# MrTornado24/FENeRF

Hardware: AMD Instinct MI355X
Metric: rays/s/GPU forward render (128x128, 24+24 samples, H=256 FiLM-SIREN + 32x96^3 grid) (higher is better)
Workload: dtype f16x3 (error-compensated fp16 MFMA, fp32 accumulate; fp32-class accuracy); 1 GPU; configs[1]: CelebA_double_semantic_texture_embedding_256_dim_96 generator, 128x128, 24+24 hierarchical samples, batch 1/GPU, forward-only render, procedural weights; img_size=128, num_steps=24, batch_per_gpu=1

## Files before the change

### fenerf_amd/csrc/fenerf_siren_f16w.hip

```cpp
#include <hip/hip_runtime.h>

#include <type_traits>

#include "fenerf_composite_ray.h"
#include "fenerf_film.h"
#include "fenerf_internal.h"
#include "fenerf_layout.h"
#include "fenerf_trig.h"


namespace fenerf {
namespace w16 {

typedef float f32x4 __attribute__((ext_vector_type(4)));
typedef _Float16 half8 __attribute__((ext_vector_type(8)));
typedef _Float16 half4 __attribute__((ext_vector_type(4)));
typedef _Float16 half2 __attribute__((ext_vector_type(2)));

#define MFMA16W(a, b, c) __builtin_amdgcn_mfma_f32_16x16x32_f16((a), (b), (c), 0, 0, 0)
#define MFMA32W(a, b, c) __builtin_amdgcn_mfma_f32_16x16x4f32((a), (b), (c), 0, 0, 0)

constexpr int CH = FENERF_CH;
constexpr int DPF = FENERF_DPF;
constexpr int NSLOT = FENERF_NSLOT;
constexpr int NWAVE = 8;
static_assert(CH == NWAVE, "one 1-KiB A operand per wave and chunk");
static_assert(NSLOT >= DPF + 2, "a slot is refilled two barriers after its last reader issued its reads");

__device__ __forceinline__ half8 as_half8(const float4& v) { return __builtin_bit_cast(half8, v); }
__device__ __forceinline__ unsigned lds_addr(const void* p) {
  return (unsigned)(size_t)(const __attribute__((address_space(3))) char*)p;
}
__device__ __forceinline__ void glds_1k(const char* g_lane, unsigned lds_uniform) {
  asm volatile(
      "s_mov_b32 m0, %1\n\t"
      "s_nop 0\n\t"
      "global_load_lds_dwordx4 %0, off"
      :
      : "v"(g_lane), "s"(lds_uniform)
      : "memory");
}
__device__ __forceinline__ void glds_1k_s(const void* g_uniform, unsigned voff, unsigned lds_uniform) {
  asm volatile(
      "s_mov_b32 m0, %2\n\t"
      "s_nop 0\n\t"
      "global_load_lds_dwordx4 %0, %1"
      :
      : "v"(voff), "s"(g_uniform), "s"(lds_uniform)
      : "memory");
}
__device__ __forceinline__ int opaque(int v) {
  asm volatile("" : "+v"(v));
  return v;
}
#define WAIT_VMCNT(n) asm volatile("s_waitcnt vmcnt(%0)" ::"n"(n) : "memory")
template <class T>
__device__ __forceinline__ T* uniform_ptr(T* p) {
  const unsigned long long v = reinterpret_cast<unsigned long long>(p);
  const unsigned lo = __builtin_amdgcn_readfirstlane((unsigned)v), hi = __builtin_amdgcn_readfirstlane((unsigned)(v >> 32));
  return reinterpret_cast<T*>(((unsigned long long)hi << 32) | lo);
}
template <int MODE> struct TapeW { const char* base; };
typedef unsigned u32x4 __attribute__((ext_vector_type(4)));
#ifndef FENERF_ST_POLICY
#define FENERF_ST_POLICY "nt"
#endif
__device__ __forceinline__ void st_f4_nt(const void* g_uniform, unsigned voff, const f32x4& v) {
  asm volatile("global_store_dwordx4 %0, %1, %2 " FENERF_ST_POLICY "\n\ts_nop 1" : : "v"(voff), "v"(v), "s"(g_uniform) : "memory");
}
__device__ __forceinline__ void st_u4_nt(const void* g_uniform, unsigned voff, const u32x4& v) {
  asm volatile("global_store_dwordx4 %0, %1, %2 " FENERF_ST_POLICY "\n\ts_nop 1" : : "v"(voff), "v"(v), "s"(g_uniform) : "memory");
}
struct TapeQ { unsigned q[4]; };
__device__ __forceinline__ unsigned phase_u16(float theta) {
  const float v = __builtin_amdgcn_fractf(theta) * 65536.f;
  const unsigned c = __builtin_bit_cast(unsigned, v + 8388608.f) & 0xffffu;
  return !(__builtin_fabsf(theta) < __builtin_inff()) ? TAPE16_NONFINITE : (c == TAPE16_NONFINITE ? (v < 65535.f ? 0xfffeu : 0u) : c);
}
#define LDS_FENCE() asm volatile("" ::: "memory")
#ifndef FENERF_WAVE_HALF_COPIES
#define FENERF_WAVE_HALF_COPIES 1
#endif
#ifndef FENERF_EXP_DEPHASE
#define FENERF_EXP_DEPHASE 0
#endif

struct WStream {
  bool skip;
  unsigned long long g_next;
  unsigned voff;
  unsigned ring_lds;
  const char* ring_lane;
  bool early;
};

__device__ __forceinline__ void ws_issue(WStream& w, int slot) {
  const unsigned m0 = w.ring_lds + (unsigned)slot * (CH * 1024);
  if (!w.skip)
    asm volatile(
        "s_mov_b32 m0, %2\n\t"
        "s_nop 0\n\t"
        "global_load_lds_dwordx4 %0, %1"
        :
        : "v"(w.voff), "s"(w.g_next), "s"(m0)
        : "memory");
  w.g_next += CH * 1024;
}

struct AK { float4 hi[2], lo[2]; };
__device__ __forceinline__ void ws_read_lo(AK& a, const WStream& w, int slot, int spl) {
  const float4* p = reinterpret_cast<const float4*>(w.ring_lane + slot * (CH * 1024) + spl * 4096);
  a.lo[0] = p[1 * 64]; a.lo[1] = p[3 * 64];
}
__device__ __forceinline__ void ws_read_hi(AK& a, const WStream& w, int slot, int spl) {
  const float4* p = reinterpret_cast<const float4*>(w.ring_lane + slot * (CH * 1024) + spl * 4096);
  a.hi[0] = p[0 * 64]; a.hi[1] = p[2 * 64];
}
template <bool LO = true>
__device__ __forceinline__ AK ws_read(const WStream& w, int slot, int spl) {
  AK a;
  if (LO) ws_read_lo(a, w, slot, spl);
  else { a.lo[0] = make_float4(0.f, 0.f, 0.f, 0.f); a.lo[1] = a.lo[0]; }
  ws_read_hi(a, w, slot, spl);
  return a;
}

__device__ __forceinline__ void ws_step(WStream& w, int i, bool early) {
  const bool sync = (i & 1) == 0;
  if (sync) {
    WAIT_VMCNT(DPF - 3);
    __builtin_amdgcn_s_barrier();
  }
  LDS_FENCE();
  if (early)
    ws_issue(w, (i + DPF) % NSLOT);
}
__device__ __forceinline__ void ws_issue_late(WStream& w, int i, bool early) {
  if (!early) ws_issue(w, (i + DPF) % NSLOT);
}

template <bool LO = true>
__device__ __forceinline__ void kstep_mfma(f32x4 (&acc)[2], const AK& a, const half8& bh, const half8& bl) {
  if (LO) {
    acc[0] = MFMA16W(as_half8(a.lo[0]), bh, acc[0]);
    acc[1] = MFMA16W(as_half8(a.lo[1]), bh, acc[1]);
  }
  acc[0] = MFMA16W(as_half8(a.hi[0]), bl, acc[0]);
  acc[1] = MFMA16W(as_half8(a.hi[1]), bl, acc[1]);
  acc[0] = MFMA16W(as_half8(a.hi[0]), bh, acc[0]);
  acc[1] = MFMA16W(as_half8(a.hi[1]), bh, acc[1]);
}

struct FilmQ { float2 f, p; };
template <int PF4>
__device__ __forceinline__ FilmQ epi_load(int nbp, int piece, const float* film) {
  const int rt = piece >> 1, pc = piece & 1;
  FilmQ q;
  q.f = *reinterpret_cast<const float2*>(film + 32 * nbp + 8 * rt + 2 * pc);
  q.p = *reinterpret_cast<const float2*>(film + PF4 + 32 * nbp + 8 * rt + 2 * pc);
  return q;
}
template <int KS, int SAVE>
__device__ __forceinline__ void epi_compute(const f32x4 (&acc)[2], int nbp, int piece, const FilmQ& q, half8 (&yh)[KS],
                                            half8 (&yl)[KS], TapeW<SAVE> tw, int tile_odd, TapeQ& tq) {
  const int rt = piece >> 1, pc = piece & 1;
  const float2 f = q.f, p = q.p;
  if (SAVE == 1 && pc == 0) {
    const int lo = opaque((int)(threadIdx.x & 63));
    const unsigned toff = (unsigned)(((2 * (lo >> 5)) * 64 + ((lo >> 4) & 1) * 32 + 16 * tile_odd + (lo & 15)) * 16);
    st_f4_nt(tw.base + (nbp * 4 + rt) * 1024, toff, acc[rt]);
  }
  const float th0 = __builtin_fmaf(f.x, acc[rt][2 * pc + 0], p.x), th1 = __builtin_fmaf(f.y, acc[rt][2 * pc + 1], p.y);
  if (SAVE == 2) {
    tq.q[piece] = __builtin_amdgcn_perm(phase_u16(th1), phase_u16(th0), 0x05040100u);
    if (piece == 3) {
      const int lo = opaque((int)(threadIdx.x & 63));
      const u32x4 v = {tq.q[0], tq.q[1], tq.q[2], tq.q[3]};
      st_u4_nt(tw.base + nbp * 2048, (unsigned)(1024 * tile_odd + 16 * lo), v);
    }
  }
  const float s0 = sin2pi(th0);
  const float s1 = sin2pi(th1);
  const _Float16 h0 = (_Float16)__builtin_fmaf(s0, F16_ACT_SCALE, 0.f), h1 = (_Float16)__builtin_fmaf(s1, F16_ACT_SCALE, 0.f);
  half2 hp = {h0, h1}, lp = {(_Float16)__builtin_fmaf(s0, F16_ACT_SCALE, -(float)h0), (_Float16)__builtin_fmaf(s1, F16_ACT_SCALE, -(float)h1)};
  asm volatile("" : "+v"(hp), "+v"(lp));
  const int s = 4 * rt + 2 * pc;
  yh[nbp][s] = hp[0]; yh[nbp][s + 1] = hp[1];
  yl[nbp][s] = lp[0]; yl[nbp][s + 1] = lp[1];
}
template <int KS, int PF4, int SAVE>
__device__ __forceinline__ void epi_piece(const f32x4 (&acc)[2], int nbp, int piece, const float* film, half8 (&yh)[KS],
                                          half8 (&yl)[KS], TapeW<SAVE> tw, int tile_odd, TapeQ& tq) {
  epi_compute<KS, SAVE>(acc, nbp, piece, epi_load<PF4>(nbp, piece, film), yh, yl, tw, tile_odd, tq);
}
template <int KS, int PF4, int SAVE>
__device__ __forceinline__ void epi_all(const f32x4 (&acc)[2], int nbp, const float* film, half8 (&yh)[KS], half8 (&yl)[KS],
                                        TapeW<SAVE> tw, int tile_odd) {
  TapeQ tq;
#pragma unroll
  for (int pc = 0; pc < 4; ++pc) epi_piece<KS, PF4, SAVE>(acc, nbp, pc, film, yh, yl, tw, tile_odd, tq);
}

struct APipe { AK c, n; };
struct FilmQ2 { FilmQ q[4]; };
template <bool LOR = true, bool LOM = true, int PH = -1, class BOP, class LOADQ, class PIECE>
__device__ __forceinline__ void chunk_step(f32x4 (&acc)[2], APipe& a, WStream& ws, int i, int sp0, BOP bop, LOADQ loadq, PIECE piece) {
  const bool early = PH < 0 ? ws.early : PH == 0;
  constexpr int PSPL = (PH == 1 && FENERF_EXP_DEPHASE == 1) ? 0 : 1;
  ws_step(ws, i, early);
  FilmQ2 fq;
#pragma unroll
  for (int spl = 0; spl < 2; ++spl) {
    if (spl == 1) ws_issue_late(ws, i, early);
    if (spl == 0) loadq(fq);
    const AK nn = ws_read<LOR>(ws, (i + 1) % NSLOT, spl);
    __builtin_amdgcn_sched_barrier(0);
    half8 bh, bl;
    if (bop(sp0 + spl, bh, bl)) kstep_mfma<LOR && LOM>(acc, a.c, bh, bl);
    if (spl == PSPL) piece(fq);
    a.c = a.n;
    a.n = nn;
    __builtin_amdgcn_sched_barrier(0);
  }
}
template <bool LO = true, int PH = -1>
__device__ __forceinline__ void chunk_skip(APipe& a, WStream& ws, int i) {
  const bool early = PH < 0 ? ws.early : PH == 0;
  ws_step(ws, i, early);
  ws_issue_late(ws, i, early);
  a.c = ws_read<LO>(ws, (i + 1) % NSLOT, 0);
  a.n = ws_read<LO>(ws, (i + 1) % NSLOT, 1);
  __builtin_amdgcn_sched_barrier(0);
}

template <int QB>
__device__ __forceinline__ void piece_range(int qc, int& p0, int& p1) {
  constexpr int QBE = QB < 4 ? QB : 4;
  if (qc >= QBE) { p0 = p1 = 0; return; }
  p0 = 4 * qc / QBE;
  p1 = 4 * (qc + 1) / QBE;
}

template <bool FUSED> struct FuseArgs {};
template <> struct FuseArgs<true> {
  int rays_per_group, octs_per_group;
  long long groups, total_rays;
  float* z_fine;
  float* out_fine;
  CompositeParams coarse;
  CompositeParams final_;
};
#ifndef FENERF_EXP_RAY_PHASE
#define FENERF_EXP_RAY_PHASE 2
#endif
#ifndef FENERF_EXP_FUSED_MAXM
#define FENERF_EXP_FUSED_MAXM 128
#endif
constexpr int FUSED_MAXM = FENERF_EXP_FUSED_MAXM;

template <int H, bool GRID, int SAVE, bool FUSED = false, int TERMS2 = 0>
__global__ __launch_bounds__(512, 2) void siren16w_kernel(SirenParams P, int n_geo, int n_color, int n_lab, int C, FuseArgs<FUSED> F) {
  static_assert(!(FUSED && SAVE != 0), "the fused render is the no-grad path");
  static_assert(TERMS2 == 0 || (SAVE == 0 && !FUSED), "the reduced-precision forwards are plain no-grad evaluations");
  constexpr bool LOR = TERMS2 != 1;
  constexpr bool LOC = TERMS2 == 0;
  constexpr int NB = H / 32, KS = H / 32;
  constexpr int QB = (KS + 1) / 2;
  constexpr int C0_KS = KS + (GRID ? 1 : 0) + 1;
  constexpr int C0_QB = (2 * (2 * KS + (GRID ? 2 : 0) + 1) + CH - 1) / CH;
  constexpr int SQ_CHUNKS = pad_stage(NB * QB * CH) / CH;
  constexpr int C0_CHUNKS = pad_stage(NB * C0_QB * CH) / CH;
  constexpr int HEAD_CHUNKS = pad_stage(QB * CH) / CH;
  extern __shared__ __attribute__((aligned(16))) float4 smem[];

  if (P.clk && threadIdx.x == 0) {
    P.clk[(size_t)blockIdx.x * 4 + 0] = __builtin_amdgcn_s_memtime();
    P.clk[(size_t)blockIdx.x * 4 + 1] = __builtin_amdgcn_s_memrealtime();
  }
  const int lane = threadIdx.x & 63;
  const int wave = __builtin_amdgcn_readfirstlane(threadIdx.x >> 6);
  const int n = lane & 15, g = lane >> 4;
  const int L = n_geo + n_color;
  const int stage_f4 = (16 * C + 3) / 4;
  char* lds = reinterpret_cast<char*>(smem);
  char* ring = lds;
  constexpr int FILM_F = H * 4 < 1024 ? 1024 : H * 4;
  constexpr int FILM_BYTES = 2 * FILM_F;
  char* film_base = lds + NSLOT * CH * 1024 + wave * (2 * FILM_BYTES);
  float* l0_lds = reinterpret_cast<float*>(lds + NSLOT * CH * 1024 + NWAVE * 2 * FILM_BYTES);
  float* cst = l0_lds + NB * 256;
  float* stage = cst + 80 + wave * stage_f4 * 4;
  float4* ext_wave = reinterpret_cast<float4*>(cst + 80 + NWAVE * stage_f4 * 4) + wave * 256;

  for (int i = threadIdx.x; i < NB * 256; i += 512) l0_lds[i] = P.stream[i];
  if (threadIdx.x < 32) {
    cst[threadIdx.x] = P.consts[CONST_FILM_BIAS + (size_t)2 * L * H + threadIdx.x];
    cst[32 + threadIdx.x] = P.consts[CONST_HEAD_BIAS + threadIdx.x];
  } else if (threadIdx.x < 36) {
    cst[64 + threadIdx.x - 32] = P.consts[CONST_FILM_BIAS + (size_t)2 * L * H + threadIdx.x];
    cst[68 + threadIdx.x - 32] = P.consts[CONST_RGB_BIAS + threadIdx.x - 32];
  }
  CompositeParams* ray_par = reinterpret_cast<CompositeParams*>(reinterpret_cast<float4*>(cst + 80 + NWAVE * stage_f4 * 4) + NWAVE * 256);
  if constexpr (FUSED) {
    constexpr int NW = (int)(sizeof(CompositeParams) / 4);
    static_assert(sizeof(CompositeParams) % 4 == 0 && NW <= 256, "copied one dword per thread");
    const int t = threadIdx.x & 255;
    const unsigned* src = reinterpret_cast<const unsigned*>(threadIdx.x < 256 ? &F.coarse : &F.final_);
    if (t < NW) reinterpret_cast<unsigned*>(ray_par + (threadIdx.x >> 8))[t] = src[t];
  }
  WAIT_VMCNT(0);
  __syncthreads();

  WStream ws;
  {
    const int spl = wave >> 2, rt = (wave >> 1) & 1, hl = wave & 1;
    const int gi = n >> 2, r = n & 3;
    const int row = 16 * (gi >> 1) + 4 * (gi & 1) + 8 * rt + r;
    const int e_old = 2 * (2 * spl + (g >> 1)) + hl;
    ws.voff = e_old * 1024 + ((g & 1) * 32 + row) * 16;
  }
  const unsigned long long g_stream = reinterpret_cast<unsigned long long>(P.stream + P.ring_offset_floats);
  ws.g_next = g_stream;
  ws.ring_lds = __builtin_amdgcn_readfirstlane(lds_addr(ring) + wave * 1024);
  ws.ring_lane = ring + lane * 16;
  ws.early = wave < NWAVE / 2;
  ws.skip = TERMS2 == 1 && (wave & 1);

  const long long ntiles = (P.P + 15) / 16;
  const long long nocts = (ntiles + NWAVE - 1) / NWAVE;
  int opg = 1;
  long long nunits = nocts;
  if constexpr (FUSED) { opg = F.octs_per_group; nunits = F.groups; }
  const int nblk = gridDim.x;
  const int nx = nblk < 8 ? nblk : 8;
  const int xcd = blockIdx.x % nx, bi = blockIdx.x / nx;
  const int blocks_in_x = nblk / nx + (xcd < nblk % nx ? 1 : 0);
  const long long o_begin = nunits * xcd / nx, o_end = nunits * (xcd + 1) / nx;

  if (P.raw_fg && o_begin + bi < o_end) {
    const long long p_first = (o_begin + bi) * opg * (NWAVE * 16);
    long long p_last = o_end * opg * (NWAVE * 16) - 1;
    if (p_last >= P.P) p_last = P.P - 1;
    film_prep_prologue(P, p_first / P.pts_per_image, p_last / P.pts_per_image, H, n_geo, n_color);
  }

#pragma unroll
  for (int i = 0; i < DPF; ++i) ws_issue(ws, i);
  WAIT_VMCNT(DPF - 1);
  __builtin_amdgcn_s_barrier();
  LDS_FENCE();
  if (wave >= NWAVE / 2) __builtin_amdgcn_s_setprio(1);
  APipe a_cur;
  a_cur.c = ws_read<LOR>(ws, 0, 0);
  a_cur.n = ws_read<LOR>(ws, 0, 1);


  for (long long unit = o_begin + bi; unit < o_end; unit += blocks_in_x) {
  const int nsub = FUSED ? 2 * opg : 1;
#pragma unroll 1
  for (int sub = 0; sub < nsub; ++sub) {
    const bool fine_pass = FUSED && sub >= opg;
    const long long oct = FUSED ? unit * opg + (fine_pass ? sub - opg : sub) : unit;
    const float* z_src = P.z;
    float* out_dst = P.out;
    if constexpr (FUSED) {
      if (fine_pass) { z_src = F.z_fine; out_dst = F.out_fine; }
    }
    ws.g_next = g_stream + (unsigned long long)DPF * (CH * 1024);
    const long long tile = oct * NWAVE + wave;
    long long pt = tile * 16 + n;
    if (pt >= P.P) pt = P.P - 1;
    const long long img = __builtin_amdgcn_readfirstlane((int)(pt / P.pts_per_image));
    float px, py, pz, dx, dy, dz;
    if (P.points) {
      px = P.points[pt * 3 + 0]; py = P.points[pt * 3 + 1]; pz = P.points[pt * 3 + 2];
      if (P.pdirs) { dx = P.pdirs[pt * 3 + 0]; dy = P.pdirs[pt * 3 + 1]; dz = P.pdirs[pt * 3 + 2]; }
      else { dx = 0.f; dy = 0.f; dz = -1.f; }
    } else {
      const long long ray = pt / P.n_per_ray;
      const float zz = z_src[pt];
      const float ox = P.origins[ray * 3 + 0], oy = P.origins[ray * 3 + 1], oz = P.origins[ray * 3 + 2];
      dx = P.dirs[ray * 3 + 0]; dy = P.dirs[ray * 3 + 1]; dz = P.dirs[ray * 3 + 2];
      px = __fadd_rn(ox, __fmul_rn(dx, zz)); py = __fadd_rn(oy, __fmul_rn(dy, zz)); pz = __fadd_rn(oz, __fmul_rn(dz, zz));
      if (P.lock_view) { dx = 0.f; dy = 0.f; dz = -1.f; }
    }
    const float qx = px * P.box_scale, qy = py * P.box_scale, qz = pz * P.box_scale;
    constexpr int TL = SAVE == 2 ? H * 64 : H * 128;
    const int tile_odd = (int)(tile & 1);
    const char* tape_tile = SAVE ? uniform_ptr(reinterpret_cast<const char*>(P.tape) + (size_t)(tile >> 1) * L * TL) : nullptr;
    auto tape_of = [&](int layer) {
      TapeW<SAVE> t{SAVE ? uniform_ptr(tape_tile + (size_t)layer * TL) : nullptr};
      if (SAVE) asm volatile("s_nop 4" ::: "memory");
      return t;
    };

    const float* fp_img = P.fp + (size_t)img * L * H;
    const float* pp_img = P.pp + (size_t)img * L * H;
    auto film_issue = [&](int layer) {
      const unsigned dst = __builtin_amdgcn_readfirstlane(lds_addr(film_base) + (layer & 1) * FILM_BYTES);
      const float* gf = fp_img + (size_t)layer * H;
      const float* gp = pp_img + (size_t)layer * H;
      const unsigned vo = (unsigned)opaque(lane) * 16;
      for (int off = 0; off < H * 4; off += 1024) {
        glds_1k_s(reinterpret_cast<const char*>(gf) + off, vo, dst + off);
        glds_1k_s(reinterpret_cast<const char*>(gp) + off, vo, dst + FILM_F + off);
      }
    };
    film_issue(0);
    if (L > 1) film_issue(1);

    float e[8];
#pragma unroll
    for (int i = 0; i < 8; ++i) e[i] = 0.f;
    if (GRID) {
      const int ch0 = 16 * (g & 1) + 8 * (g >> 1);
      const float ix = ((qx + 1.f) / 2.f) * (float)(P.gw - 1);
      const float iy = ((qy + 1.f) / 2.f) * (float)(P.gh - 1);
      const float iz = ((qz + 1.f) / 2.f) * (float)(P.gd - 1);
      const float x0 = floorf(ix), y0 = floorf(iy), z0 = floorf(iz);
#pragma unroll
      for (int c = 0; c < 8; ++c) {
        const int cz = c >> 2, cy = (c >> 1) & 1, cx = c & 1;
        const float xi = x0 + cx, yi = y0 + cy, zi = z0 + cz;
        const float wx = cx ? (ix - x0) : (x0 + 1.f - ix);
        const float wy = cy ? (iy - y0) : (y0 + 1.f - iy);
        const float wz = cz ? (iz - z0) : (z0 + 1.f - iz);
        const float wgt = wx * wy * wz;
        const bool ok = xi >= 0.f && xi <= (float)(P.gw - 1) && yi >= 0.f && yi <= (float)(P.gh - 1) && zi >= 0.f &&
                        zi <= (float)(P.gd - 1);
        if (ok) {
          const long long vox = ((long long)(int)zi * P.gh + (int)yi) * P.gw + (int)xi;
          const float4* gp = reinterpret_cast<const float4*>(P.grid + vox * 32 + ch0);
#pragma unroll
          for (int q = 0; q < 2; ++q) {
            const float4 v = gp[q];
            e[4 * q + 0] += v.x * wgt; e[4 * q + 1] += v.y * wgt; e[4 * q + 2] += v.z * wgt; e[4 * q + 3] += v.w * wgt;
          }
        }
      }
    }
    if (SAVE && GRID) {
      float4* ep = reinterpret_cast<float4*>(P.tape_e + pt * 32 + 16 * (g & 1) + 8 * (g >> 1));
      ep[0] = make_float4(e[0], e[1], e[2], e[3]);
      ep[1] = make_float4(e[4], e[5], e[6], e[7]);
    }
    {
      half8 eh, el, dh, dl;
#pragma unroll
      for (int t = 0; t < 8; ++t) {
        const float v = e[t] * F16_ACT_SCALE;
        const _Float16 hh = (_Float16)v;
        eh[t] = hh; el[t] = (_Float16)(v - (float)hh);
      }
      const float d3[3] = {dx * F16_ACT_SCALE, dy * F16_ACT_SCALE, dz * F16_ACT_SCALE};
#pragma unroll
      for (int t = 0; t < 8; ++t) { dh[t] = (_Float16)0.f; dl[t] = (_Float16)0.f; }
#pragma unroll
      for (int t = 0; t < 3; ++t) {
        const float v = g == 0 ? d3[t] : 0.f;
        const _Float16 hh = (_Float16)v;
        dh[t] = hh; dl[t] = (_Float16)(v - (float)hh);
      }
      float4* ext = ext_wave + lane;
      ext[0] = __builtin_bit_cast(float4, eh); ext[64] = __builtin_bit_cast(float4, el);
      ext[128] = __builtin_bit_cast(float4, dh); ext[192] = __builtin_bit_cast(float4, dl);
    }
    WAIT_VMCNT(0);
    LDS_FENCE();

    auto film_lane = [&](int layer) -> const float* {
      const int gq = opaque(lane) >> 4;
      return reinterpret_cast<const float*>(film_base + (layer & 1) * FILM_BYTES) + 16 * (gq >> 1) + 4 * (gq & 1);
    };

    half8 xh[KS], xl[KS];
    {
      const float b = g == 0 ? qx : (g == 1 ? qy : (g == 2 ? qz : 0.f));
      const int gi = n >> 2, r = n & 3;
      const float* wl = l0_lds + ((g & 1) * 32 + 16 * (gi >> 1) + 4 * (gi & 1) + r) * 4 + (g >> 1);
      const TapeW<SAVE> tw0 = tape_of(0);
#pragma unroll
      for (int nb = 0; nb < NB; ++nb) {
        f32x4 acc[2];
#pragma unroll
        for (int rt = 0; rt < 2; ++rt) {
          const f32x4 z4 = {0.f, 0.f, 0.f, 0.f};
          acc[rt] = MFMA32W(wl[nb * 256 + 8 * rt * 4], b, z4);
        }
        epi_all<KS, FILM_F / 4, SAVE>(acc, nb, film_lane(0), xh, xl, tw0, tile_odd);
      }
    }
    auto film_layer = [&](auto ph_c, int l) {
      constexpr int PH = decltype(ph_c)::value;
      const float* ff = film_lane(l);
      const TapeW<SAVE> tw = tape_of(l);
      half8 yh[KS], yl[KS];
      if (l + 1 < L) film_issue(l + 1);
      if (SQ_CHUNKS < DPF + 2) WAIT_VMCNT(0);
      if (l == n_geo) {
        const float4* ext = ext_wave + opaque(lane);
        auto bop0 = [&](int sp, half8& bh, half8& bl) -> bool {
          if (sp < KS) { bh = xh[sp]; bl = xl[sp]; return true; }
          if (GRID && sp == KS) { bh = as_half8(ext[0]); bl = as_half8(ext[64]); return true; }
          if (sp == C0_KS - 1) { bh = as_half8(ext[128]); bl = as_half8(ext[192]); return true; }
          return false;
        };
        f32x4 acc_prev[2] = {{0.f, 0.f, 0.f, 0.f}, {0.f, 0.f, 0.f, 0.f}};
        TapeQ tq;
#pragma unroll
        for (int nb = 0; nb < NB; ++nb) {
          f32x4 acc[2] = {{0.f, 0.f, 0.f, 0.f}, {0.f, 0.f, 0.f, 0.f}};
#pragma unroll
          for (int qc = 0; qc < C0_QB; ++qc) {
            chunk_step<LOR, LOC, PH>(acc, a_cur, ws, nb * C0_QB + qc, 2 * qc, bop0, [&](FilmQ2& fq) {
              if (nb > 0) {
                int p0, p1;
                piece_range<C0_QB>(qc, p0, p1);
#pragma unroll
                for (int pc = 0; pc < 4; ++pc)
                  if (pc >= p0 && pc < p1) fq.q[pc] = epi_load<FILM_F / 4>(nb - 1, pc, ff);
              }
            }, [&](const FilmQ2& fq) {
              if (nb > 0) {
                int p0, p1;
                piece_range<C0_QB>(qc, p0, p1);
#pragma unroll
                for (int pc = 0; pc < 4; ++pc)
                  if (pc >= p0 && pc < p1) epi_compute<KS, SAVE>(acc_prev, nb - 1, pc, fq.q[pc], yh, yl, tw, tile_odd, tq);
              }
            });
          }
          acc_prev[0] = acc[0]; acc_prev[1] = acc[1];
        }
#pragma unroll
        for (int i = NB * C0_QB; i < C0_CHUNKS; ++i) chunk_skip<LOR, PH>(a_cur, ws, i);
        epi_all<KS, FILM_F / 4, SAVE>(acc_prev, NB - 1, ff, yh, yl, tw, tile_odd);
        {
          f32x4 acc[2] = {{0.f, 0.f, 0.f, 0.f}, {0.f, 0.f, 0.f, 0.f}};
          auto bop = [&](int sp, half8& bh, half8& bl) -> bool {
            if (sp < KS) { bh = xh[sp]; bl = xl[sp]; return true; }
            return false;
          };
#pragma unroll
          for (int qc = 0; qc < QB; ++qc) chunk_step<LOR, true, PH>(acc, a_cur, ws, qc, 2 * qc, bop, [](FilmQ2&) {}, [](const FilmQ2&) {});
#pragma unroll
          for (int i = QB; i < HEAD_CHUNKS; ++i) chunk_skip<LOR, PH>(a_cur, ws, i);
          const int lane_o = opaque(lane);
          const int n_o = lane_o & 15, f_o = 16 * (lane_o >> 5) + 4 * ((lane_o >> 4) & 1);
#pragma unroll
          for (int rt = 0; rt < 2; ++rt) {
#pragma unroll
            for (int r = 0; r < 4; ++r) {
              const int row = f_o + 8 * rt + r;
              if (row <= n_lab) {
                const int ch = row < n_lab ? row : C - 1;
                stage[n_o * C + ch] = acc[rt][r] * cst[row] + cst[32 + row];
              }
            }
          }
        }
      } else {
        auto square_stage = [&](auto lom_c) {
        constexpr bool LOM = decltype(lom_c)::value;
        auto bop = [&](int sp, half8& bh, half8& bl) -> bool {
          if (sp < KS) { bh = xh[sp]; bl = xl[sp]; return true; }
          return false;
        };
        f32x4 acc_prev[2] = {{0.f, 0.f, 0.f, 0.f}, {0.f, 0.f, 0.f, 0.f}};
        TapeQ tq;
#pragma unroll
        for (int nb = 0; nb < NB; ++nb) {
          f32x4 acc[2] = {{0.f, 0.f, 0.f, 0.f}, {0.f, 0.f, 0.f, 0.f}};
#pragma unroll
          for (int qc = 0; qc < QB; ++qc) {
            chunk_step<LOR, LOM, PH>(acc, a_cur, ws, nb * QB + qc, 2 * qc, bop, [&](FilmQ2& fq) {
              if (nb > 0) {
                int p0, p1;
                piece_range<QB>(qc, p0, p1);
#pragma unroll
                for (int pc = 0; pc < 4; ++pc)
                  if (pc >= p0 && pc < p1) fq.q[pc] = epi_load<FILM_F / 4>(nb - 1, pc, ff);
              }
            }, [&](const FilmQ2& fq) {
              if (nb > 0) {
                int p0, p1;
                piece_range<QB>(qc, p0, p1);
#pragma unroll
                for (int pc = 0; pc < 4; ++pc)
                  if (pc >= p0 && pc < p1) epi_compute<KS, SAVE>(acc_prev, nb - 1, pc, fq.q[pc], yh, yl, tw, tile_odd, tq);
              }
            });
          }
          acc_prev[0] = acc[0]; acc_prev[1] = acc[1];
        }
#pragma unroll
        for (int i = NB * QB; i < SQ_CHUNKS; ++i) chunk_skip<LOR, PH>(a_cur, ws, i);
        epi_all<KS, FILM_F / 4, SAVE>(acc_prev, NB - 1, ff, yh, yl, tw, tile_odd);
        };
        if constexpr (TERMS2 == 2) {
          if (l < n_geo) square_stage(std::true_type{}); else square_stage(std::false_type{});
        } else {
          square_stage(std::integral_constant<bool, LOR>{});
        }
      }
#pragma unroll
      for (int k = 0; k < KS; ++k) { xh[k] = yh[k]; xl[k] = yl[k]; }
    };
#pragma unroll 1
    for (int l = 1; l < L; ++l) {
#if FENERF_WAVE_HALF_COPIES
      if (ws.early) film_layer(std::integral_constant<int, 0>{}, l); else film_layer(std::integral_constant<int, 1>{}, l);
#else
      film_layer(std::integral_constant<int, -1>{}, l);
#endif
    }
    {
      constexpr int PH = -1;
      f32x4 acc[2] = {{0.f, 0.f, 0.f, 0.f}, {0.f, 0.f, 0.f, 0.f}};
      auto bop = [&](int sp, half8& bh, half8& bl) -> bool {
        if (sp < KS) { bh = xh[sp]; bl = xl[sp]; return true; }
        return false;
      };
#pragma unroll
      for (int qc = 0; qc < QB; ++qc) chunk_step<LOR, LOC, PH>(acc, a_cur, ws, qc, 2 * qc, bop, [](FilmQ2&) {}, [](const FilmQ2&) {});
#pragma unroll
      for (int i = QB; i < HEAD_CHUNKS; ++i) chunk_skip<LOR, PH>(a_cur, ws, i);
      const int lane_o = opaque(lane);
      const int n_o = lane_o & 15;
      if ((lane_o >> 4) == 0) {
#pragma unroll
        for (int r = 0; r < 3; ++r) {
          const float v = acc[0][r] * cst[64 + r] + cst[68 + r];
          stage[n_o * C + (C - 4) + r] = 1.f / (1.f + __expf(-v));
        }
      }
    }
    __builtin_amdgcn_fence(__ATOMIC_RELEASE, "wavefront");
    __builtin_amdgcn_wave_barrier();
    __builtin_amdgcn_fence(__ATOMIC_ACQUIRE, "wavefront");
    {
      const long long base = tile * 16 * C;
      const long long limit = P.P * C;
      for (int i = opaque(lane); i < 16 * C; i += 64)
        if (base + i < limit) out_dst[base + i] = stage[i];
    }
    WAIT_VMCNT(0);
    __builtin_amdgcn_wave_barrier();
    if constexpr (FUSED) {
      if (FENERF_EXP_RAY_PHASE > 0 && (sub == opg - 1 || sub == nsub - 1)) {
        __builtin_amdgcn_fence(__ATOMIC_RELEASE, "workgroup");
        __builtin_amdgcn_s_barrier();
        __builtin_amdgcn_fence(__ATOMIC_ACQUIRE, "workgroup");
        float* sc = reinterpret_cast<float*>(ext_wave);
        float* s_z = sc;
        float* s_zs = sc + FUSED_MAXM;
        int* s_ord = reinterpret_cast<int*>(sc + 2 * FUSED_MAXM + 4);
        float* s_w = sc + 3 * FUSED_MAXM + 4;
        const int lane_r = opaque(lane);
        const long long ray0 = unit * F.rays_per_group;
        for (int r = wave; r < F.rays_per_group; r += NWAVE) {
          const long long ray = ray0 + r;
          if (FENERF_EXP_RAY_PHASE > 1 && ray < F.total_rays) {
#pragma unroll 1
            for (int rep = 0; rep < (FENERF_EXP_RAY_PHASE > 2 ? 2 : 1); ++rep) {
              if (!fine_pass) composite_ray<false, FUSED_MAXM>(ray_par[0], ray, lane_r, s_z, s_zs, s_ord, s_w);
              else composite_ray<true, FUSED_MAXM>(ray_par[1], ray, lane_r, s_z, s_zs, s_ord, s_w);
              __builtin_amdgcn_wave_barrier();
            }
          }
          __builtin_amdgcn_wave_barrier();
        }
        if (!fine_pass) {
          __builtin_amdgcn_fence(__ATOMIC_RELEASE, "workgroup");
          __builtin_amdgcn_s_barrier();
          __builtin_amdgcn_fence(__ATOMIC_ACQUIRE, "workgroup");
        }
        WAIT_VMCNT(0);
      }
    }
  }
  }
  WAIT_VMCNT(0);
  __builtin_amdgcn_s_barrier();
  if (P.clk && threadIdx.x == 0) {
    P.clk[(size_t)blockIdx.x * 4 + 2] = __builtin_amdgcn_s_memtime();
    P.clk[(size_t)blockIdx.x * 4 + 3] = __builtin_amdgcn_s_memrealtime();
  }
}

static int hip_fail16w(hipError_t e, const char* what) {
  set_error(std::string(what) + ": " + hipGetErrorString(e));
  return FENERF_E_HIP;
}

static size_t lds_bytes_16w(const FenerfModel* m, int H) {
  const int stage_f4 = (16 * m->C + 3) / 4;
  const size_t film_f = H * 4 < 1024 ? 1024 : H * 4;
  return (size_t)NSLOT * CH * 1024 + (size_t)NWAVE * 2 * (2 * film_f) + (size_t)(H / 32) * 1024 + 80 * 4 +
         (size_t)NWAVE * stage_f4 * 16 + (size_t)NWAVE * 4096;
}

template <int H, bool GRID>
static int launch_fused_t(const FenerfModel* m, const SirenParams& p, const FuseArgs<true>& F, int blocks, void* stream) {
  const size_t lds = lds_bytes_16w(m, H) + (2 * sizeof(CompositeParams) + 255) / 256 * 256;
  auto kfn = siren16w_kernel<H, GRID, 0, true>;
  if (int rc = ensure_dynamic_lds(reinterpret_cast<const void*>(kfn), lds)) return rc;
  hipLaunchKernelGGL(kfn, dim3((unsigned)blocks), dim3(512), lds, (hipStream_t)stream, p, m->n_geo, m->n_color, m->n_lab, m->C, F);
  hipError_t e = hipGetLastError();
  return e == hipSuccess ? FENERF_OK : hip_fail16w(e, "fused render launch");
}

template <int H, bool GRID, int SAVE, int TERMS2 = 0>
static int launch_t(const FenerfModel* m, const SirenParams& p, void* stream) {
  const size_t lds = lds_bytes_16w(m, H);
  auto kfn = siren16w_kernel<H, GRID, SAVE, false, TERMS2>;
  if (int rc = ensure_dynamic_lds(reinterpret_cast<const void*>(kfn), lds)) return rc;
  const long long ntiles = (p.P + 15) / 16;
  long long blocks = (ntiles + NWAVE - 1) / NWAVE;
  if (blocks > m->num_cus) blocks = m->num_cus;
  if (blocks < 1) blocks = 1;
  hipLaunchKernelGGL(kfn, dim3((unsigned)blocks), dim3(512), lds, (hipStream_t)stream, p, m->n_geo, m->n_color, m->n_lab, m->C, FuseArgs<false>{});
  hipError_t e = hipGetLastError();
  return e == hipSuccess ? FENERF_OK : hip_fail16w(e, "siren16w launch");
}

}

static int launch_siren16w_one(const FenerfModel* m, const SirenParams& q, void* stream) {
  const bool g = m->grid_ch != 0;
  if (q.tape && q.tape_format == FENERF_TAPE_U16) {
    switch (m->H) {
      case 32: return g ? w16::launch_t<32, true, 2>(m, q, stream) : w16::launch_t<32, false, 2>(m, q, stream);
      case 64: return g ? w16::launch_t<64, true, 2>(m, q, stream) : w16::launch_t<64, false, 2>(m, q, stream);
      case 96: return g ? w16::launch_t<96, true, 2>(m, q, stream) : w16::launch_t<96, false, 2>(m, q, stream);
      case 128: return g ? w16::launch_t<128, true, 2>(m, q, stream) : w16::launch_t<128, false, 2>(m, q, stream);
      case 192: return g ? w16::launch_t<192, true, 2>(m, q, stream) : w16::launch_t<192, false, 2>(m, q, stream);
      case 256: return g ? w16::launch_t<256, true, 2>(m, q, stream) : w16::launch_t<256, false, 2>(m, q, stream);
    }
  }
  if (q.tape) {
    switch (m->H) {
      case 32: return g ? w16::launch_t<32, true, 1>(m, q, stream) : w16::launch_t<32, false, 1>(m, q, stream);
      case 64: return g ? w16::launch_t<64, true, 1>(m, q, stream) : w16::launch_t<64, false, 1>(m, q, stream);
      case 96: return g ? w16::launch_t<96, true, 1>(m, q, stream) : w16::launch_t<96, false, 1>(m, q, stream);
      case 128: return g ? w16::launch_t<128, true, 1>(m, q, stream) : w16::launch_t<128, false, 1>(m, q, stream);
      case 192: return g ? w16::launch_t<192, true, 1>(m, q, stream) : w16::launch_t<192, false, 1>(m, q, stream);
      case 256: return g ? w16::launch_t<256, true, 1>(m, q, stream) : w16::launch_t<256, false, 1>(m, q, stream);
    }
  }
  if (m->forward_mode == FENERF_FORWARD_F16X2) {
    switch (m->H) {
      case 32: return g ? w16::launch_t<32, true, 0, 1>(m, q, stream) : w16::launch_t<32, false, 0, 1>(m, q, stream);
      case 64: return g ? w16::launch_t<64, true, 0, 1>(m, q, stream) : w16::launch_t<64, false, 0, 1>(m, q, stream);
      case 96: return g ? w16::launch_t<96, true, 0, 1>(m, q, stream) : w16::launch_t<96, false, 0, 1>(m, q, stream);
      case 128: return g ? w16::launch_t<128, true, 0, 1>(m, q, stream) : w16::launch_t<128, false, 0, 1>(m, q, stream);
      case 192: return g ? w16::launch_t<192, true, 0, 1>(m, q, stream) : w16::launch_t<192, false, 0, 1>(m, q, stream);
      case 256: return g ? w16::launch_t<256, true, 0, 1>(m, q, stream) : w16::launch_t<256, false, 0, 1>(m, q, stream);
    }
  }
  if (m->forward_mode == FENERF_FORWARD_F16X3_COLOR_X2) {
    switch (m->H) {
      case 32: return g ? w16::launch_t<32, true, 0, 2>(m, q, stream) : w16::launch_t<32, false, 0, 2>(m, q, stream);
      case 64: return g ? w16::launch_t<64, true, 0, 2>(m, q, stream) : w16::launch_t<64, false, 0, 2>(m, q, stream);
      case 96: return g ? w16::launch_t<96, true, 0, 2>(m, q, stream) : w16::launch_t<96, false, 0, 2>(m, q, stream);
      case 128: return g ? w16::launch_t<128, true, 0, 2>(m, q, stream) : w16::launch_t<128, false, 0, 2>(m, q, stream);
      case 192: return g ? w16::launch_t<192, true, 0, 2>(m, q, stream) : w16::launch_t<192, false, 0, 2>(m, q, stream);
      case 256: return g ? w16::launch_t<256, true, 0, 2>(m, q, stream) : w16::launch_t<256, false, 0, 2>(m, q, stream);
    }
  }
  switch (m->H) {
    case 32: return g ? w16::launch_t<32, true, 0>(m, q, stream) : w16::launch_t<32, false, 0>(m, q, stream);
    case 64: return g ? w16::launch_t<64, true, 0>(m, q, stream) : w16::launch_t<64, false, 0>(m, q, stream);
    case 96: return g ? w16::launch_t<96, true, 0>(m, q, stream) : w16::launch_t<96, false, 0>(m, q, stream);
    case 128: return g ? w16::launch_t<128, true, 0>(m, q, stream) : w16::launch_t<128, false, 0>(m, q, stream);
    case 192: return g ? w16::launch_t<192, true, 0>(m, q, stream) : w16::launch_t<192, false, 0>(m, q, stream);
    case 256: return g ? w16::launch_t<256, true, 0>(m, q, stream) : w16::launch_t<256, false, 0>(m, q, stream);
  }
  set_error("unsupported hidden_dim");
  return FENERF_E_UNSUPPORTED;
}

bool fused_render_plan(const FenerfModel* m, long long B, long long R, int N, bool balanced_only, FusedRenderPlan* plan) {
  if (m->precision != FENERF_PREC_F16X3 || N < 3 || 2 * N > w16::FUSED_MAXM) return false;
  if (m->forward_mode != FENERF_FORWARD_F16X3) return false;
  int g = N, b = 128;
  while (b) { const int t = g % b; g = b; b = t; }
  const int G = 128 / g, opg = N / g;
  if (R % G != 0) return false;
  const long long groups = B * R / G, nocts = groups * opg;
  const long long cus = launch_cus(m);
  const long long blocks_f = groups < cus ? groups : cus, blocks_p = nocts < cus ? nocts : cus;
  if (balanced_only && (groups + blocks_f - 1) / blocks_f * opg > (nocts + blocks_p - 1) / blocks_p) return false;
  plan->rays_per_group = G; plan->octs_per_group = opg; plan->groups = groups; plan->blocks = (int)blocks_f;
  return true;
}

int launch_render16w_fused(const FenerfModel* m, const SirenParams& p, const FusedRenderPlan& plan, float* z_fine, float* out_fine,
                           const CompositeParams& coarse, const CompositeParams& final_, void* stream) {
  w16::FuseArgs<true> F;
  F.rays_per_group = plan.rays_per_group; F.octs_per_group = plan.octs_per_group; F.groups = plan.groups;
  F.total_rays = coarse.BR;
  F.z_fine = z_fine; F.out_fine = out_fine; F.coarse = coarse; F.final_ = final_;
  const bool g = m->grid_ch != 0;
  switch (m->H) {
    case 32: return g ? w16::launch_fused_t<32, true>(m, p, F, plan.blocks, stream) : w16::launch_fused_t<32, false>(m, p, F, plan.blocks, stream);
    case 64: return g ? w16::launch_fused_t<64, true>(m, p, F, plan.blocks, stream) : w16::launch_fused_t<64, false>(m, p, F, plan.blocks, stream);
    case 96: return g ? w16::launch_fused_t<96, true>(m, p, F, plan.blocks, stream) : w16::launch_fused_t<96, false>(m, p, F, plan.blocks, stream);
    case 128: return g ? w16::launch_fused_t<128, true>(m, p, F, plan.blocks, stream) : w16::launch_fused_t<128, false>(m, p, F, plan.blocks, stream);
    case 192: return g ? w16::launch_fused_t<192, true>(m, p, F, plan.blocks, stream) : w16::launch_fused_t<192, false>(m, p, F, plan.blocks, stream);
    case 256: return g ? w16::launch_fused_t<256, true>(m, p, F, plan.blocks, stream) : w16::launch_fused_t<256, false>(m, p, F, plan.blocks, stream);
  }
  set_error("unsupported hidden_dim");
  return FENERF_E_UNSUPPORTED;
}

int launch_siren16w(const FenerfModel* m, const SirenParams& p, void* stream) {
  if (p.P <= 0) return FENERF_OK;
  if (p.pts_per_image % 32 == 0 || p.P == p.pts_per_image) return launch_siren16w_one(m, p, stream);
  const long long nimg = p.P / p.pts_per_image;
  const int L = m->L, H = m->H;
  for (long long b = 0; b < nimg; ++b) {
    SirenParams q = p;
    q.P = p.pts_per_image;
    q.fp = p.fp + (size_t)b * L * H;
    q.pp = p.pp + (size_t)b * L * H;
    if (p.raw_fg) {
      q.raw_fg = p.raw_fg + (size_t)b * m->n_geo * H; q.raw_pg = p.raw_pg + (size_t)b * m->n_geo * H;
      q.raw_fa = p.raw_fa + (size_t)b * m->n_color * H; q.raw_pa = p.raw_pa + (size_t)b * m->n_color * H;
      q.n_images = 1;
    }
    q.out = p.out + (size_t)b * p.pts_per_image * m->C;
    if (p.points) {
      q.points = p.points + (size_t)b * p.pts_per_image * 3;
      if (p.pdirs) q.pdirs = p.pdirs + (size_t)b * p.pts_per_image * 3;
    } else {
      const long long rays = p.pts_per_image / p.n_per_ray;
      q.origins = p.origins + (size_t)b * rays * 3;
      q.dirs = p.dirs + (size_t)b * rays * 3;
      q.z = p.z + (size_t)b * p.pts_per_image;
    }
    int rc = launch_siren16w_one(m, q, stream);
    if (rc) return rc;
  }
  return FENERF_OK;
}

}
```

Baseline: 6.020 million rays/s.

## Defer last FiLM epilogue block into next layer's MFMA chunks

Moves the final output-block FiLM/sine epilogue of each SIREN layer out of the layer tail and spreads it across the first chunk steps of the next layer (and the head), so the epilogue ALU work overlaps the next layer's MFMAs and weight streaming. The next layer's film prefetch is delayed until the deferred pieces have been issued. Layer 0 is restructured to batch all MFMAs first and double-buffer film loads with sched barriers. Branches are made opaque/scalar via readfirstlane flags so both variants of the layer body are not merged. This raises register pressure (acc_last and the extra film buffers) and adds code size, which risks spills at 512-thread launch bounds.

Measured after the change: 6.108 million rays/s, median of 6. +1.5%, better.

```diff
diff --git a/fenerf_amd/csrc/fenerf_siren_f16w.hip b/fenerf_amd/csrc/fenerf_siren_f16w.hip
--- a/fenerf_amd/csrc/fenerf_siren_f16w.hip
+++ b/fenerf_amd/csrc/fenerf_siren_f16w.hip
@@ -54,6 +54,11 @@
   return v;
 }
 #define WAIT_VMCNT(n) asm volatile("s_waitcnt vmcnt(%0)" ::"n"(n) : "memory")
+__device__ __forceinline__ bool opaque_flag(bool b) {
+  int v = b;
+  asm volatile("" : "+v"(v));
+  return __builtin_amdgcn_readfirstlane(v) != 0;
+}
 template <class T>
 __device__ __forceinline__ T* uniform_ptr(T* p) {
   const unsigned long long v = reinterpret_cast<unsigned long long>(p);
@@ -271,6 +276,8 @@
   constexpr int SQ_CHUNKS = pad_stage(NB * QB * CH) / CH;
   constexpr int C0_CHUNKS = pad_stage(NB * C0_QB * CH) / CH;
   constexpr int HEAD_CHUNKS = pad_stage(QB * CH) / CH;
+  constexpr bool DEFER = QB >= 2;
+  constexpr int QBD = !DEFER ? 1 : (QB - 1 < 4 ? QB - 1 : 4);
   extern __shared__ __attribute__((aligned(16))) float4 smem[];
 
   if (P.clk && threadIdx.x == 0) {
@@ -474,30 +481,81 @@
     };
 
     half8 xh[KS], xl[KS];
+    f32x4 acc_last[2];
+    auto defer_load = [&](FilmQ2& fq, int qc, const float* ffd) {
+      if (DEFER) {
+        int p0, p1;
+        piece_range<QBD>(qc, p0, p1);
+#pragma unroll
+        for (int pc = 0; pc < 4; ++pc)
+          if (pc >= p0 && pc < p1) fq.q[pc] = epi_load<FILM_F / 4>(NB - 1, pc, ffd);
+      }
+    };
+    auto defer_run = [&](const FilmQ2& fq, int qc, TapeW<SAVE> twd, TapeQ& tq) {
+      if (DEFER) {
+        int p0, p1;
+        piece_range<QBD>(qc, p0, p1);
+#pragma unroll
+        for (int pc = 0; pc < 4; ++pc)
+          if (pc >= p0 && pc < p1) epi_compute<KS, SAVE>(acc_last, NB - 1, pc, fq.q[pc], xh, xl, twd, tile_odd, tq);
+      }
+    };
     {
       const float b = g == 0 ? qx : (g == 1 ? qy : (g == 2 ? qz : 0.f));
       const int gi = n >> 2, r = n & 3;
       const float* wl = l0_lds + ((g & 1) * 32 + 16 * (gi >> 1) + 4 * (gi & 1) + r) * 4 + (g >> 1);
       const TapeW<SAVE> tw0 = tape_of(0);
+      float w0[NB][2];
+      f32x4 acc0[NB][2];
+#pragma unroll
+      for (int nb = 0; nb < NB; ++nb) { w0[nb][0] = wl[nb * 256]; w0[nb][1] = wl[nb * 256 + 8 * 4]; }
+      constexpr int NBE = DEFER ? NB - 1 : NB;
+      const float* ff0 = film_lane(0);
+      FilmQ2 fq[2];
+#pragma unroll
+      for (int pc = 0; pc < 4; ++pc) fq[0].q[pc] = epi_load<FILM_F / 4>(0, pc, ff0);
+      __builtin_amdgcn_sched_barrier(0);
 #pragma unroll
       for (int nb = 0; nb < NB; ++nb) {
-        f32x4 acc[2];
 #pragma unroll
         for (int rt = 0; rt < 2; ++rt) {
           const f32x4 z4 = {0.f, 0.f, 0.f, 0.f};
-          acc[rt] = MFMA32W(wl[nb * 256 + 8 * rt * 4], b, z4);
+          acc0[nb][rt] = MFMA32W(w0[nb][rt], b, z4);
         }
-        epi_all<KS, FILM_F / 4, SAVE>(acc, nb, film_lane(0), xh, xl, tw0, tile_odd);
-      }
+      }
+      __builtin_amdgcn_sched_barrier(0);
+#pragma unroll
+      for (int nb = 0; nb < NBE; ++nb) {
+        if (nb + 1 < NBE) {
+#pragma unroll
+          for (int pc = 0; pc < 4; ++pc) fq[(nb + 1) & 1].q[pc] = epi_load<FILM_F / 4>(nb + 1, pc, ff0);
+        }
+        __builtin_amdgcn_sched_barrier(0);
+        TapeQ tq;
+#pragma unroll
+        for (int pc = 0; pc < 4; ++pc) epi_compute<KS, SAVE>(acc0[nb], nb, pc, fq[nb & 1].q[pc], xh, xl, tw0, tile_odd, tq);
+        __builtin_amdgcn_sched_barrier(0);
+      }
+      if (DEFER) { acc_last[0] = acc0[NB - 1][0]; acc_last[1] = acc0[NB - 1][1]; }
     }
     auto film_layer = [&](auto ph_c, int l) {
       constexpr int PH = decltype(ph_c)::value;
       const float* ff = film_lane(l);
       const TapeW<SAVE> tw = tape_of(l);
       half8 yh[KS], yl[KS];
-      if (l + 1 < L) film_issue(l + 1);
+      const float* ffd = DEFER ? film_lane(l - 1) : nullptr;
+      const TapeW<SAVE> twd = DEFER ? tape_of(l - 1) : TapeW<SAVE>{nullptr};
+      if (!DEFER && l + 1 < L) film_issue(l + 1);
+      auto film_issue_deferred = [&](int i) {
+        if (DEFER && i == QBD - 1 && l + 1 < L) film_issue(l + 1);
+      };
       if (SQ_CHUNKS < DPF + 2) WAIT_VMCNT(0);
-      if (l == n_geo) {
+      auto x_gets_y = [&]() {
+#pragma unroll
+        for (int k = 0; k < (DEFER ? KS - 1 : KS); ++k) { xh[k] = yh[k]; xl[k] = yl[k]; }
+      };
+      const bool is_c0 = opaque_flag(l == n_geo), is_sq = opaque_flag(l != n_geo);
+      if (is_c0) {
         const float4* ext = ext_wave + opaque(lane);
         auto bop0 = [&](int sp, half8& bh, half8& bl) -> bool {
           if (sp < KS) { bh = xh[sp]; bl = xl[sp]; return true; }
@@ -519,7 +577,7 @@
 #pragma unroll
                 for (int pc = 0; pc < 4; ++pc)
                   if (pc >= p0 && pc < p1) fq.q[pc] = epi_load<FILM_F / 4>(nb - 1, pc, ff);
-              }
+              } else defer_load(fq, qc, ffd);
             }, [&](const FilmQ2& fq) {
               if (nb > 0) {
                 int p0, p1;
@@ -527,14 +585,16 @@
 #pragma unroll
                 for (int pc = 0; pc < 4; ++pc)
                   if (pc >= p0 && pc < p1) epi_compute<KS, SAVE>(acc_prev, nb - 1, pc, fq.q[pc], yh, yl, tw, tile_odd, tq);
-              }
+              } else defer_run(fq, qc, twd, tq);
             });
+            if (nb == 0) film_issue_deferred(qc);
           }
           acc_prev[0] = acc[0]; acc_prev[1] = acc[1];
         }
 #pragma unroll
         for (int i = NB * C0_QB; i < C0_CHUNKS; ++i) chunk_skip<LOR, PH>(a_cur, ws, i);
-        epi_all<KS, FILM_F / 4, SAVE>(acc_prev, NB - 1, ff, yh, yl, tw, tile_odd);
+        if (DEFER) { acc_last[0] = acc_prev[0]; acc_last[1] = acc_prev[1]; }
+        else epi_all<KS, FILM_F / 4, SAVE>(acc_prev, NB - 1, ff, yh, yl, tw, tile_odd);
         {
           f32x4 acc[2] = {{0.f, 0.f, 0.f, 0.f}, {0.f, 0.f, 0.f, 0.f}};
           auto bop = [&](int sp, half8& bh, half8& bl) -> bool {
@@ -559,7 +619,9 @@
             }
           }
         }
-      } else {
+        x_gets_y();
+      }
+      if (is_sq) {
         auto square_stage = [&](auto lom_c) {
         constexpr bool LOM = decltype(lom_c)::value;
         auto bop = [&](int sp, half8& bh, half8& bl) -> bool {
@@ -580,7 +642,7 @@
 #pragma unroll
                 for (int pc = 0; pc < 4; ++pc)
                   if (pc >= p0 && pc < p1) fq.q[pc] = epi_load<FILM_F / 4>(nb - 1, pc, ff);
-              }
+              } else defer_load(fq, qc, ffd);
             }, [&](const FilmQ2& fq) {
               if (nb > 0) {
                 int p0, p1;
@@ -588,28 +650,33 @@
 #pragma unroll
                 for (int pc = 0; pc < 4; ++pc)
                   if (pc >= p0 && pc < p1) epi_compute<KS, SAVE>(acc_prev, nb - 1, pc, fq.q[pc], yh, yl, tw, tile_odd, tq);
-              }
+              } else defer_run(fq, qc, twd, tq);
             });
+            if (nb == 0) film_issue_deferred(qc);
           }
           acc_prev[0] = acc[0]; acc_prev[1] = acc[1];
         }
 #pragma unroll
         for (int i = NB * QB; i < SQ_CHUNKS; ++i) chunk_skip<LOR, PH>(a_cur, ws, i);
-        epi_all<KS, FILM_F / 4, SAVE>(acc_prev, NB - 1, ff, yh, yl, tw, tile_odd);
+        if (DEFER) { acc_last[0] = acc_prev[0]; acc_last[1] = acc_prev[1]; }
+        else epi_all<KS, FILM_F / 4, SAVE>(acc_prev, NB - 1, ff, yh, yl, tw, tile_odd);
+        x_gets_y();
         };
         if constexpr (TERMS2 == 2) {
-          if (l < n_geo) square_stage(std::true_type{}); else square_stage(std::false_type{});
+          const bool geo = opaque_flag(l < n_geo), col = opaque_flag(l >= n_geo);
+          if (geo) square_stage(std::true_type{});
+          if (col) square_stage(std::false_type{});
         } else {
           square_stage(std::integral_constant<bool, LOR>{});
         }
       }
-#pragma unroll
-      for (int k = 0; k < KS; ++k) { xh[k] = yh[k]; xl[k] = yl[k]; }
     };
 #pragma unroll 1
     for (int l = 1; l < L; ++l) {
 #if FENERF_WAVE_HALF_COPIES
-      if (ws.early) film_layer(std::integral_constant<int, 0>{}, l); else film_layer(std::integral_constant<int, 1>{}, l);
+      const bool half0 = opaque_flag(ws.early), half1 = opaque_flag(!ws.early);
+      if (half0) film_layer(std::integral_constant<int, 0>{}, l);
+      if (half1) film_layer(std::integral_constant<int, 1>{}, l);
 #else
       film_layer(std::integral_constant<int, -1>{}, l);
 #endif
@@ -621,8 +688,13 @@
         if (sp < KS) { bh = xh[sp]; bl = xl[sp]; return true; }
         return false;
       };
-#pragma unroll
-      for (int qc = 0; qc < QB; ++qc) chunk_step<LOR, LOC, PH>(acc, a_cur, ws, qc, 2 * qc, bop, [](FilmQ2&) {}, [](const FilmQ2&) {});
+      const float* ffd = DEFER ? film_lane(L - 1) : nullptr;
+      const TapeW<SAVE> twd = DEFER ? tape_of(L - 1) : TapeW<SAVE>{nullptr};
+      TapeQ tq;
+#pragma unroll
+      for (int qc = 0; qc < QB; ++qc)
+        chunk_step<LOR, LOC, PH>(acc, a_cur, ws, qc, 2 * qc, bop, [&](FilmQ2& fq) { defer_load(fq, qc, ffd); },
+                                 [&](const FilmQ2& fq) { defer_run(fq, qc, twd, tq); });
 #pragma unroll
       for (int i = QB; i < HEAD_CHUNKS; ++i) chunk_skip<LOR, PH>(a_cur, ws, i);
       const int lane_o = opaque(lane);
```
